# rensonnetg/microstructure_fingerprinting

Hardware: AMD Instinct MI355X
Metric: voxels/sec, 2-fascicle exhaustive NNLS, 782-atom x 200-measurement dictionary (higher is better)
Workload: dtype f64 (pairs ranked on split-f16 MFMA, short list re-evaluated in f64); 1 GPU; C2: 100000 voxels/GPU, 2 fascicles, 782 atoms x 200 measurements; voxels_per_gpu=100000, global_voxels=100000, atoms=782, measurements=200, ranks_in_group=1

## Files before the change

### microstructure_fingerprinting_amd/csrc/fit_k2.hip

```cpp
#pragma once
#include <type_traits>

#include "mfx_device.h"
#include "nnls_small.h"

typedef double d4 __attribute__((ext_vector_type(4)));

#define MFX_WG 512
#define MFX_MAXC 256
#define MFX_S_CAP 2048
#define MFX_DET_REL 1e-8
#define MFX_A12_REL 4e-14

struct FitK2Args {
  TablesDev T;
  PlanDev P;
  const double* Y;
  const double* peaks;
  int peaks_ld;
  const int* vox_list;
  const int* list_count;
  double* params;
  int num_params;
  int maxfasc;
  int csf_on, ear_on;
  unsigned long long* stamps;
  int* fb_count;
  int* fb_list;
  int maxc;
  int scap;
  const double* xc;
  struct Cand* xl_cand;
  int* xl_cnt;
  double* xl_mrg;
  int xl_cap;
  int vox_base;
  int* audit;
};

#ifdef MFX_STAMPS
#define MFX_STAMP(i) do { if (a.stamps && tid == 0) a.stamps[(size_t)blockIdx.x * 16 + (i)] = __builtin_amdgcn_s_memtime(); } while (0)
#else
#define MFX_STAMP(i) do { } while (0)
#endif

struct Cand {
  double score;
  int i, j;
};

__device__ __forceinline__ double wave_max(double v) {
#pragma unroll
  for (int o = 32; o > 0; o >>= 1) v = fmax(v, __shfl_xor(v, o));
  return v;
}
__device__ __forceinline__ double wave_sum(double v) {
#pragma unroll
  for (int o = 32; o > 0; o >>= 1) v += __shfl_xor(v, o);
  return v;
}

template <int I, int N, typename F>
__device__ __forceinline__ void mfx_static_for(F&& f) {
  if constexpr (I < N) {
    f(std::integral_constant<int, I>{});
    mfx_static_for<I + 1, N>(f);
  }
}

template <int KSTEPS, bool BRACKET, bool PIPE, int NW = 8, int TILES = 2, int NBUF = 2>
__global__ __launch_bounds__(NW * 64, NW == 8 ? 2 : 1) void mfx_fit_k2_kernel(FitK2Args a) {
  constexpr bool FAST = PIPE && !BRACKET;
  constexpr int WG = NW * 64;
  static_assert(!FAST || (NW == 8 && TILES == 2 && NBUF == 2), "the pipelined path is written for 8 waves, 2 tiles, 2 buffers");
  static_assert(TILES == 1 || TILES == 2, "TILES");
  static_assert(NBUF == 1 || NBUF == 2, "NBUF");
  constexpr int MP = KSTEPS * 4;
  constexpr int MPS = ((MP + 15) / 16) * 16;
  extern __shared__ double smem[];
  const int tid = threadIdx.x, lane = tid & 63, wave = tid >> 6;
  const int lg = lane >> 4, lc = lane & 15;
  const int M = a.P.M, N = a.T.N, ldn = a.T.ldn;
  const int NP = ldn;
  const int ntiles = NP >> 4;
  const double2* __restrict__ tab = a.T.tab;
  if (a.list_count && (int)blockIdx.x >= *a.list_count) return;
  const int vox = a.vox_list ? a.vox_list[blockIdx.x] : blockIdx.x;

  double* sB = smem;
  double* s_y = sB + NBUF * TILES * MPS * 16;
  double* s_t0 = s_y + MP;
  double* s_t1 = s_t0 + 2 * MP;
  double* s_tG = s_t1 + (BRACKET ? 2 * MP : 0);
  double* s_dG = s_tG + (BRACKET ? MP : 0);
  double* s_A11 = s_dG + (BRACKET ? MP : 0);
  double* s_Y1 = s_A11 + NP;
  double* s_A22 = s_Y1 + NP;
  double* s_Y2 = s_A22 + NP;
  double* s_S2 = s_Y2 + NP;
  double* s_S1 = s_S2 + NP;
  double* s_red = s_S1 + NP;
  Cand* s_cand = (Cand*)(s_red + 32);
  int* s_r0 = (int*)(s_cand + MFX_MAXC);
  int* s_r1 = s_r0 + 2 * MP;
  int* s_cnt = s_r1 + (BRACKET ? 2 * MP : 0);

  MFX_STAMP(0);
  const double* __restrict__ yv = a.Y + (size_t)vox * M;
  const double* __restrict__ pk = a.peaks + (size_t)vox * a.peaks_ld;
  for (int m = tid; m < MP; m += WG) s_y[m] = (m < M) ? yv[m] : 0.0;
  for (int idx = tid; idx < 2 * MP; idx += WG) {
    const int k = idx / MP, m = idx - k * MP;
    RowDesc rd;
    rd.r0 = a.T.P; rd.t0 = 0.0; rd.r1 = -1; rd.t1 = 0.0;
    if (m < M) rd = mfx_row_desc(a.T, a.P, m, pk[3 * k], pk[3 * k + 1], pk[3 * k + 2]);
    s_r0[idx] = rd.r0;
    s_t0[idx] = rd.t0;
    if (BRACKET) {
      s_r1[idx] = rd.r1;
      s_t1[idx] = rd.t1;
      if (k == 0) { s_tG[m] = (m < M) ? a.P.tG[m] : 0.0; s_dG[m] = (m < M) ? a.P.dG[m] : 1.0; }
    }
  }
  if (tid == 0) s_cnt[0] = 0;
  if (tid < 2) mfx_check_dir(a.P, pk + 3 * tid, vox);
  __syncthreads();

  auto elem = [&](int k, int m, int n) -> double {
    if (BRACKET) {
      RowDesc rd;
      rd.r0 = s_r0[k * MP + m]; rd.t0 = s_t0[k * MP + m];
      rd.r1 = s_r1[k * MP + m]; rd.t1 = s_t1[k * MP + m];
      return mfx_eval_br(tab, ldn, rd, s_tG[m], s_dG[m], n);
    } else {
      return mfx_eval(tab, ldn, s_r0[k * MP + m], s_t0[k * MP + m], n);
    }
  };

  MFX_STAMP(1);
  double y_sq = 0.0;
  for (int m = 0; m < M; ++m) y_sq += s_y[m] * s_y[m];
  double my_s[2] = {0.0, 0.0};
  int my_n[2] = {0, 0};
  for (int col = tid; col < 2 * NP; col += WG) {
    const int k = col >= NP, n = col - k * NP;
    double a2 = 0.0, ay = 0.0;
    if (n < N) {
#pragma unroll 8
      for (int m = 0; m < M; ++m) {
        if constexpr (FAST) {
          const double2 e = tab[(size_t)s_r0[k * MP + m] * ldn + n];
          const double d = fma(e.y, s_t0[k * MP + m], e.x);
          a2 = fma(d, d, a2);
          ay = fma(s_y[m], d, ay);
        } else {
          const double d = elem(k, m, n);
          a2 += d * d;
          ay += s_y[m] * d;
        }
      }
    }
    if constexpr (FAST) {
      const double inv = (n < N && a2 > 0.0) ? 1.0 / sqrt(a2) : 0.0;
      const double z = ay * inv;
      (k ? s_A22 : s_A11)[n] = inv;
      (k ? s_Y2 : s_Y1)[n] = z;
      const double s = z > 0.0 ? z * z : 0.0;
      if (s > my_s[k]) { my_s[k] = s; my_n[k] = n; }
    } else {
      (k ? s_A22 : s_A11)[n] = a2;
      (k ? s_Y2 : s_Y1)[n] = ay;
      const double s = (n < N && ay > 0.0) ? (ay * ay) / a2 : 0.0;
      (k ? s_S2 : s_S1)[n] = s;
      if (s > my_s[k]) { my_s[k] = s; my_n[k] = n; }
    }
  }
  const double eps_abs = 1e-9 * y_sq;
  double glb_run = 0.0;
  {
    double* s_bs = s_red;
    int* s_bn = (int*)(s_red + 16);
#pragma unroll
    for (int k = 0; k < 2; ++k) {
      double s = my_s[k];
      int n = my_n[k];
#pragma unroll
      for (int o = 32; o > 0; o >>= 1) {
        const double s2 = __shfl_xor(s, o);
        const int n2 = __shfl_xor(n, o);
        const bool take = (s2 > s) || (s2 == s && n2 < n);
// ... 422 lines not shown
```

### microstructure_fingerprinting_amd/csrc/fit_k2s.hip

```cpp
#pragma once
#include "fit_k2.hip"

typedef _Float16 h8 __attribute__((ext_vector_type(8)));
typedef _Float16 h4 __attribute__((ext_vector_type(4)));
typedef float f32x16 __attribute__((ext_vector_type(16)));
typedef float f32x2 __attribute__((ext_vector_type(2)));
typedef float f32x4 __attribute__((ext_vector_type(4)));
typedef int i32x4 __attribute__((ext_vector_type(4)));

#ifndef MFX_S_DC
#define MFX_S_DC 1.5e-5
#endif
template <int KS>
__host__ __device__ constexpr double mfx_s_dc() { return KS <= 13 ? (double)MFX_S_DC : 1.05 * (2.38e-6 + 3.0 * KS * 3.046e-7); }
#define MFX_S_DENMIN 1e-3
#define MFX_S_BOUND 0x40000000
#define MFX_S_GUARD 0.25

__device__ __forceinline__ unsigned long long mfx_nonneg_bits(double x) {
  return (unsigned long long)__double_as_longlong(x > 0.0 ? x : 0.0);
}

template <int CTRL>
__device__ __forceinline__ float mfx_dpp_max_f32(float v) {
  const int o = __builtin_amdgcn_update_dpp(0, __float_as_int(v), CTRL, 0xf, 0xf, false);
  return fmaxf(v, __int_as_float(o));
}
__device__ __forceinline__ double mfx_wave_max_down(double x) {
  float v = (float)x * (1.0f - 1.2e-7f);
  v = mfx_dpp_max_f32<0xb1>(v);
  v = mfx_dpp_max_f32<0x4e>(v);
  v = mfx_dpp_max_f32<0x141>(v);
  v = mfx_dpp_max_f32<0x140>(v);
  const int b = __float_as_int(v);
  const float r0 = __int_as_float(__builtin_amdgcn_readlane(b, 0)), r1 = __int_as_float(__builtin_amdgcn_readlane(b, 16)),
              r2 = __int_as_float(__builtin_amdgcn_readlane(b, 32)), r3 = __int_as_float(__builtin_amdgcn_readlane(b, 48));
  return (double)fmaxf(fmaxf(r0, r1), fmaxf(r2, r3));
}
__device__ __forceinline__ double mfx_rcp_nr(double x) {
  const double r0 = (double)__builtin_amdgcn_rcpf((float)x);
  return fma(r0, fma(-x, r0, 1.0), r0);
}

__device__ __forceinline__ double mfx_readlane_f64(double v, int l) {
  const long long b = __double_as_longlong(v);
  const unsigned lo = (unsigned)__builtin_amdgcn_readlane((int)(b & 0xffffffffll), l);
  const unsigned hi = (unsigned)__builtin_amdgcn_readlane((int)(b >> 32), l);
  return __longlong_as_double((long long)(((unsigned long long)hi << 32) | lo));
}

__device__ __forceinline__ void mfx_split16(float f, _Float16& hi, _Float16& lo) {
  asm("" : "+v"(f));
  const float h = __uint_as_float(__float_as_uint(f) & 0xffffe000u);
  hi = (_Float16)h;
  lo = (_Float16)(f - h);
}

#include "k2s_shared.h"

template <int KS, bool BR = false, int NB = 3, bool XC = false>
__global__ __launch_bounds__(512, 2) void mfx_fit_k2s_kernel(FitK2Args a) {
  constexpr int WG = 512, NW = 8;
  constexpr int MP = KS * 16;
  extern __shared__ double smem[];
  int tid = threadIdx.x;
  const int lane = tid & 63, wave = tid >> 6;
  const int lr = lane & 31, lh = lane >> 5;
  [[maybe_unused]] const int M = a.P.M;
  const int N = a.T.N, ldn = a.T.ldn;
  const int NP = (N + 31) & ~31;
  const int ntiles = NP >> 5;
  const int vox = a.vox_list ? a.vox_list[a.vox_base + blockIdx.x] : a.vox_base + (int)blockIdx.x;

  const K2sLds<KS, NB, BR, XC, NW * 64> L(smem, NP);
  K2S_UNPACK(L);
  const K2sVoxel VX = k2s_prologue<KS, NB, BR, XC, NW * 64, WG>(a, L, vox, tid);
  const double y_sq = VX.y_sq, yx = VX.yx, ramp = VX.ramp, dc_eff = VX.dc_eff, mrg = VX.mrg, etol = VX.etol;
  (void)y_sq; (void)yx;
  const float2* __restrict__ tab32 = a.P.tab32s;
  auto tab32_at = [&](int ro, int n) -> float2 { return *(const float2*)((const char*)tab32 + ((unsigned)(ro + n) << 3)); };
  auto tab32x2_at = [&](int ro, int n) -> f32x4 { return *(const f32x4*)((const char*)tab32 + ((unsigned)(ro + n) << 3)); };
  auto push = [&](double S, int i, int j) { k2s_push(L, a.scap, S, i, j); };

  MFX_STAMP(2);
#ifdef MFX_STAMPS_RND
  if (a.stamps && tid == 0) a.stamps[(size_t)blockIdx.x * 16] = __builtin_amdgcn_s_memtime();
#endif
  double bs1 = 0.0;
  int bn1 = 0;
  const int nrounds = (ntiles + NW - 1) / NW;
#ifdef MFX_EXP_NOAUDIT
  const int aud_key = -1;
#else
  const int aud_key = a.audit ? k2s_audit_key(k2s_audit_hash(vox), (ntiles % NW == 1 && ntiles > 1) ? ntiles - 1 : ntiles, ntiles) : -1;
#endif
  for (int round = 0; round < nrounds; ++round) {
    const bool tail = (ntiles - round * NW == 1) && (ntiles > 1);
    const int rt = tail ? round * NW : round * NW + wave;
    const bool rt_valid = rt < ntiles;
    const int rtc = rt_valid ? rt : 0;
    h8 afh[KS], afl[KS];
    {
      const int n = rtc * 32 + lr;
      const int nn = min(n, ldn - 1);
      double a2 = 0.0, ay = 0.0;
      float um1 = 0.0f;
      if constexpr (XC) um1 = (rt_valid && n < N) ? -s_uf[n] : 0.0f;
      mfx_static_for<0, KS>([&](auto kc) {
        constexpr int ks = decltype(kc)::value;
        float2 d[8];
#pragma unroll
        for (int j = 0; j < 8; ++j) d[j] = tab32_at(s_rs[16 * ks + 8 * lh + j], nn);
        h8 vh, vl;
#pragma unroll
        for (int j = 0; j < 8; ++j) {
          float fv = fmaf(d[j].y, s_t0f[16 * ks + 8 * lh + j], d[j].x);
          fv = rt_valid ? fv : 0.0f;
          if constexpr (XC) {
            if constexpr (ks == KS - 1) { if (j == 7) fv = lh ? um1 : fv; }
          } else {
            const double fd = (double)fv;
            a2 = fma(fd, fd, a2);
            ay = fma((double)s_yf[16 * ks + 8 * lh + j], fd, ay);
          }
          _Float16 x, y;
          mfx_split16(fv, x, y);
          vh[j] = x; vl[j] = y;
        }
        asm volatile("" : "+v"(vh), "+v"(vl));
        afh[ks] = vh; afl[ks] = vl;
        __builtin_amdgcn_sched_barrier(0);
      });
      if constexpr (!XC) {
      a2 += __shfl_xor(a2, 32);
      ay += __shfl_xor(ay, 32);
      const bool act = rt_valid && n < N;
      const double nrm = sqrt(a2);
      const double inv = (act && a2 > 0.0) ? 1.0 / nrm : 0.0;
      const double z = ay * inv;
      if (rt_valid && lh == 0) {
        s_Zf[n] = act ? (float)z : -1e30f;
        s_cs[n] = (act && a2 > 0.0) ? (float)nrm : 0.0f;
      }
      double sb = (act && z > 0.0) ? z * z : 0.0;
      int nb = n;
#pragma unroll
      for (int o = 16; o > 0; o >>= 1) {
        const double s2 = __shfl_xor(sb, o);
        const int n2 = __shfl_xor(nb, o);
        const bool take = (s2 > sb) || (s2 == sb && n2 < nb);
        sb = take ? s2 : sb;
        nb = take ? n2 : nb;
      }
      sb = mfx_readlane_f64(sb, 0);
      nb = __builtin_amdgcn_readfirstlane(nb);
      if (sb > bs1 || (sb == bs1 && sb > 0.0 && nb < bn1)) { bs1 = sb; bn1 = nb; }
      if (lane == 0 && sb - mrg > 0.0) atomicMax(&s_thr[0], mfx_nonneg_bits(sb - mrg));
      }
    }

    double thr = 0.0, thr_rows = -1.0;
#ifdef MFX_STAMPS_RND
    int dbg_flagged = 0, dbg_groups = 0;
#endif
    const float DCF = XC ? (float)((mfx_s_dc<KS>() + 2e-6) * ramp) * (1.0f + 2e-7f)
                         : (float)mfx_s_dc<KS>() + 2e-6f;
    auto pq_of = [&](float z, float rth, float& P, float& Q) {
      P = fminf(1.0f, fmaxf(z, 0.0f) * rth);
      Q = __builtin_amdgcn_sqrtf(fmaxf(0.0f, fmaf(-P, P, 1.0f) - 1.2e-7f)) * (1.0f - 3e-7f);
    };
    unsigned long long sc_thr = 0ull;
    float sc_z2 = 0.0f, sc_s = 0.0f;
    auto scan_pre = [&](int ct) {
      const int j = ct * 32 + lr;
      sc_thr = s_thr[0];
      sc_z2 = s_Zf[NP + j];
      sc_s = s_cs[NP + j];
    };
#ifdef MFX_STAMPS_SCAN
    int dbg_calls = 0;
#define MFX_SCAN_T(k) do { if (a.stamps && round == 0 && dbg_calls == 1 && wave == 0 && lane == 0) a.stamps[(size_t)blockIdx.x * 16 + (k)] = __builtin_amdgcn_s_memtime(); } while (0)
#else
#define MFX_SCAN_T(k) do { } while (0)
#endif
    auto scan_main = [&](const f32x16& acc, int ct) {
#ifdef MFX_STAMPS_SCAN
      ++dbg_calls;
#endif
      MFX_SCAN_T(0);
      {
        if (((rt << 8) | ct) == aud_key) {
          const unsigned h = k2s_audit_hash(vox);
          const int ga = (h >> 16) & 15;
          float v = acc[0];
#pragma unroll
          for (int g = 1; g < 16; ++g) v = (ga == g) ? acc[g] : v;
          if (lane == (int)((h >> 20) & 63)) ((float*)(s_red + 30))[0] = v;
        }
      }
      const int j = ct * 32 + lr;
      thr = fmax(thr, __longlong_as_double((long long)sc_thr));
      const float rth = __builtin_amdgcn_rsqf(fmaxf((float)thr * (1.0f - 2e-7f), 1e-30f)) * (1.0f + 4e-7f);
      float* pqw = s_pq + wave * 64;
      if (thr > thr_rows) {
        thr_rows = thr;
        if (lane < 32) {
          const float z1 = s_Zf[rtc * 32 + lane], n1 = s_cs[rtc * 32 + lane];
          float P, Q;
          pq_of(z1, rth, P, Q);
          const bool ok = n1 > 0.0f;
          pqw[lane] = ok ? (P + DCF) * n1 : 0.0f;
          pqw[32 + lane] = ok ? Q * ((1.0f - DCF) * n1) : 1e18f;
        }
      }
      const float z2f = sc_z2, n2 = sc_s;
      float P2, Q2;
      pq_of(z2f, rth, P2, Q2);
      const bool colok = n2 > 0.0f;
      const float p2 = colok ? (P2 + DCF) * n2 : -1e18f, q2 = colok ? Q2 * ((1.0f - DCF) * n2) : 1e18f;
      float mm[4];
#pragma unroll
      for (int q = 0; q < 4; ++q) {
        const f32x4 p1q = *(const f32x4*)(pqw + 8 * q + 4 * lh);
        const f32x4 q1q = *(const f32x4*)(pqw + 32 + 8 * q + 4 * lh);
        float t[4];
#pragma unroll
        for (int u = 0; u < 4; ++u) t[u] = fmaf(-q1q[u], q2, fmaf(p1q[u], p2, -acc[4 * q + u]));
        mm[q] = fmaxf(fmaxf(t[0], t[1]), fmaxf(t[2], t[3]));
      }
      MFX_SCAN_T(1);
      if (__any(fmaxf(fmaxf(mm[0], mm[1]), fmaxf(mm[2], mm[3])) >= 0.0f)) {
        MFX_SCAN_T(2);
#ifdef MFX_STAMPS_RND
        ++dbg_flagged;
#endif
        const double z2 = (double)s_Zf[NP + j], n2d = (double)s_cs[NP + j];
#pragma unroll 1
        for (int q = 0; q < 4; ++q) {
          if (!__any(mm[q] >= 0.0f)) continue;
          const f32x4 p1q = *(const f32x4*)(pqw + 8 * q + 4 * lh);
          const f32x4 q1q = *(const f32x4*)(pqw + 32 + 8 * q + 4 * lh);
#pragma unroll 1
          for (int gg = 0; gg < 4; ++gg) {
            const int g = 4 * q + gg;
            if (!__any(fmaf(-q1q[gg], q2, fmaf(p1q[gg], p2, -acc[g])) >= 0.0f)) continue;
#ifdef MFX_STAMPS_RND
            ++dbg_groups;
#endif
            const int i = rt * 32 + (g & 3) + 8 * (g >> 2) + 4 * lh;
            const double n12 = (double)s_cs[i] * n2d;
            const double c = n12 > 0.0 ? (double)acc[g] * mfx_rcp_nr(n12) : 0.0;
            const double z1 = (double)s_Zf[i];
            const double e1 = fma(-c, z2, z1);
            const double e2 = fma(-c, z1, z2);
            const double den = fma(-c, c, 1.0);
            const double num = fma(z2, e2, z1 * e1);
            const bool pos = (e1 > -etol) & (e2 > -etol);
            const bool wellc = (den >= MFX_S_DENMIN) & (c >= 0.0);
            const bool hit = pos & wellc & (fma(-thr, den, num) >= 0.0);
            const bool near = pos & !wellc;
            if (!__any(hit | near)) continue;
            double S = -1.0;
            if (hit) {
              S = num * mfx_rcp_nr(den);
            } else if (near) {
              const double dlo = den - 2.0 * dc_eff - dc_eff * dc_eff;
              const double u1 = fabs(e1) + etol, u2 = fabs(e2) + etol;
              S = (dlo > 0.0 && c > -0.5) ? fmin(fma(z2, z2, u1 * u1 / dlo), fma(z1, z1, u2 * u2 / dlo)) + mrg : 1e300;
            }
            bool feas = hit;
            double q1x = 0.0, q2x = 0.0;
            if constexpr (XC) {
              q1x = (double)s_uf[i] * mfx_rcp_nr(fmax((double)s_cs[i], 1e-300));
              q2x = (double)s_uf[NP + j] * mfx_rcp_nr(fmax(n2d, 1e-300));
              feas = hit && (fma(-e2, q2x, fma(-e1, q1x, yx * den)) >= 8.0 * etol);
            }
            double sraise = feas ? S : 0.0;
            double slist = S;
            if constexpr (XC) {
              if (__any(hit && !feas)) {
                const double n1p = (double)s_cs[i], u1 = (double)s_uf[i], u2 = (double)s_uf[NP + j];
                const double m1 = fma(u1, u1, n1p * n1p), m2 = fma(u2, u2, n2d * n2d);
                const double i1 = mfx_rcp_nr(fmax(sqrt(m1), 1e-300)), i2 = mfx_rcp_nr(fmax(sqrt(m2), 1e-300));
                const double w1 = fma(u1, yx, z1 * n1p) * i1, w2 = fma(u2, yx, z2 * n2d) * i2;
                const double c0 = fma(u1, u2, (double)acc[g]) * i1 * i2;
                const double f1 = fma(-c0, w2, w1), f2 = fma(-c0, w1, w2), den0 = fma(-c0, c0, 1.0);
                const bool ok0 = hit && !feas && (f1 > etol) && (f2 > etol) && (den0 >= MFX_S_DENMIN) && (c0 >= 0.0) && (m1 > 0.0) && (m2 > 0.0);
                if (ok0) sraise = fma(w2, f2, w1 * f1) * mfx_rcp_nr(den0) - yx * yx;
                const bool xneg = hit && (e1 > etol) && (e2 > etol) && (fma(-e2, q2x, fma(-e1, q1x, yx * den)) <= -8.0 * etol) &&
                                  (den0 >= MFX_S_DENMIN) && (c0 >= 0.0) && (m1 > 0.0) && (m2 > 0.0);
                if (xneg) {
                  if (ok0) slist = sraise + mrg;
                  else if (f1 < -etol || f2 < -etol) slist = -1.0;
                }
              }
            }
            const double smax = mfx_wave_max_down(fmax(sraise, 0.0));
            if (smax - 2.0 * mrg > thr) {
              thr = smax - 2.0 * mrg;
              if (lane == 0) atomicMax(&s_thr[0], mfx_nonneg_bits(thr));
            }
            if ((hit | near) && slist >= thr) push(slist, i, hit ? j : (j | MFX_S_BOUND));
#ifdef MFX_STAMPS_SCAN
            if (a.stamps && round == 0 && dbg_calls == 1 && wave == 0 && lane == 0) {
              unsigned long long* st = a.stamps + (size_t)blockIdx.x * 16;
              if (st[15] < 8) st[4 + st[15]] = __builtin_amdgcn_s_memtime();
              ++st[15];
            }
#endif
          }
        }
        MFX_SCAN_T(3);
      }
    };
    auto scan_tile = [&](const f32x16& acc, int ct) { scan_pre(ct); scan_main(acc, ct); };

#ifdef MFX_EXP_NOTAIL
    if (tail) continue;
#endif
    if (tail) {
#ifdef MFX_STAMPS_RND
      if (a.stamps && tid == 0 && round < 4) a.stamps[(size_t)blockIdx.x * 16 + 2 * round + 1] = __builtin_amdgcn_s_memtime();
#endif
      thr = __longlong_as_double((long long)s_thr[0]);
      for (int ct = wave; ct < ntiles; ct += NW) {
        const int n = ct * 32 + lr;
        const int nn = min(n, ldn - 1);
        float tail_u2 = 0.0f;
        if constexpr (XC) tail_u2 = s_uf[NP + n];
        f32x16 acc;
#pragma unroll
        for (int g = 0; g < 16; ++g) acc[g] = 0.0f;
        float2 d[2][8];
#pragma unroll
        for (int j = 0; j < 8; ++j) d[0][j] = tab32_at(s_rs[MP + 8 * lh + j], nn);
        mfx_static_for<0, KS>([&](auto kc) {
          constexpr int ks = decltype(kc)::value;
          if constexpr (ks + 1 < KS) {
#pragma unroll
            for (int j = 0; j < 8; ++j) d[(ks + 1) & 1][j] = tab32_at(s_rs[MP + 16 * (ks + 1) + 8 * lh + j], nn);
          }
          h8 bh, bl;
#pragma unroll
          for (int j = 0; j < 8; ++j) {
            _Float16 x, y;
            float fv = fmaf(d[ks & 1][j].y, s_t0f[MP + 16 * ks + 8 * lh + j], d[ks & 1][j].x);
            if constexpr (XC && ks == KS - 1) { if (j == 7) fv = lh ? tail_u2 : fv; }
            mfx_split16(fv, x, y);
            bh[j] = x; bl[j] = y;
          }
          acc = __builtin_amdgcn_mfma_f32_32x32x16_f16(afh[ks], bh, acc, 0, 0, 0);
          acc = __builtin_amdgcn_mfma_f32_32x32x16_f16(afh[ks], bl, acc, 0, 0, 0);
          acc = __builtin_amdgcn_mfma_f32_32x32x16_f16(afl[ks], bh, acc, 0, 0, 0);
          __builtin_amdgcn_sched_barrier(0);
        });
        scan_tile(acc, ct);
      }
      __syncthreads();
#ifdef MFX_STAMPS_RND
      if (a.stamps && tid == 0 && round < 4) a.stamps[(size_t)blockIdx.x * 16 + 2 * round + 2] = __builtin_amdgcn_s_memtime();
#endif
      continue;
    }

    const int grp = wave >> 2, tg = tid & 255;
    static_assert(KS <= 16, "one generation item per thread");
    f32x4 gd[8];
    const int gq = KS * grp + (tg >> 4);
    const bool gact = (tg >> 4) < KS;
    auto gen_load = [&](int ch) {
      const int nn = min(ch * 32 + 2 * (tg & 15), ldn - 2);
      const int q = gact ? gq : KS * grp;
#pragma unroll
      for (int e = 0; e < 8; ++e) gd[e] = tab32x2_at(s_rs[MP + 8 * q + e], nn);
    };
#ifndef MFX_XC_GT
#define MFX_XC_GT 0
#endif
    constexpr bool GT = KS <= 13 && (!XC || MFX_XC_GT);
    float g_t[GT ? 8 : 1];
    if constexpr (GT) {
#pragma unroll
      for (int e = 0; e < 8; ++e) g_t[e] = s_t0f[MP + 8 * (gact ? gq : KS * grp) + e];
    }
    auto gen_store = [&](int ch, int buf) {
      if (gact) {
        const int c0 = 2 * (tg & 15);
        h8 hi0, lo0, hi1, lo1;
        float gu0 = 0.0f, gu1 = 0.0f;
        if constexpr (XC) { gu0 = s_uf[NP + ch * 32 + c0]; gu1 = s_uf[NP + ch * 32 + c0 + 1]; }
#pragma unroll
        for (int e = 0; e < 8; ++e) {
          const float t = GT ? g_t[GT ? e : 0] : s_t0f[MP + 8 * gq + e];
          _Float16 x, y;
          float v0 = fmaf(gd[e][1], t, gd[e][0]), v1 = fmaf(gd[e][3], t, gd[e][2]);
          if constexpr (XC) { if (e == 7) { const bool spare = (gq == 2 * KS - 1); v0 = spare ? gu0 : v0; v1 = spare ? gu1 : v1; } }
          mfx_split16(v0, x, y);
          hi0[e] = x; lo0[e] = y;
          mfx_split16(v1, x, y);
          hi1[e] = x; lo1[e] = y;
        }
        const int off = (gq * 32 + c0) << 3;
        _Float16* dh = sBh + buf * KS * 512 + off;
        _Float16* dl = sBl + buf * KS * 512 + off;
        *(h8*)dh = hi0; *(h8*)(dh + 8) = hi1;
        *(h8*)dl = lo0; *(h8*)(dl + 8) = lo1;
      }
    };
    f32x16 acc;
#pragma unroll
    for (int g = 0; g < 16; ++g) acc[g] = 0.0f;
    auto mfma_chunk = [&](int buf) {
#pragma unroll
      for (int g = 0; g < 16; ++g) acc[g] = 0.0f;
      const _Float16* bhp = sBh + buf * KS * 512 + lane * 8;
      const _Float16* blp = sBl + buf * KS * 512 + lane * 8;
      h8 bh = *(const h8*)bhp, bl = *(const h8*)blp;
      mfx_static_for<0, KS>([&](auto kc) {
        constexpr int ks = decltype(kc)::value;
        h8 bhn = bh, bln = bl;
        if constexpr (ks + 1 < KS) {
          bhn = *(const h8*)(bhp + (ks + 1) * 512);
          bln = *(const h8*)(blp + (ks + 1) * 512);
        }
        acc = __builtin_amdgcn_mfma_f32_32x32x16_f16(afh[ks], bh, acc, 0, 0, 0);
        acc = __builtin_amdgcn_mfma_f32_32x32x16_f16(afh[ks], bl, acc, 0, 0, 0);
        acc = __builtin_amdgcn_mfma_f32_32x32x16_f16(afl[ks], bh, acc, 0, 0, 0);
        bh = bhn; bl = bln;
        __builtin_amdgcn_sched_barrier(0);
      });
    };

    if (round == 0) MFX_STAMP(3);
#ifdef MFX_STAMPS_RND
    if (a.stamps && tid == 0 && round < 4) a.stamps[(size_t)blockIdx.x * 16 + 2 * round + 1] = __builtin_amdgcn_s_memtime();
#endif
    if constexpr (NB == 3) {
      gen_load(0);
      gen_store(0, 0);
      if (grp == 0) {
        if (ntiles > 1) { gen_load(1); gen_store(1, 1); }
        if (ntiles > 2) gen_load(2);
      } else if (ntiles > 1) {
        gen_load(1);
      }
      __syncthreads();
      if (round == 0) MFX_STAMP(4);
      thr = __longlong_as_double((long long)s_thr[0]);
      int b0 = 0;
#ifdef MFX_EXP_NOGEN
      const bool exp_gen = round == 0;
#else
      constexpr bool exp_gen = true;
#endif
      for (int c = 0; c <= ntiles; ++c) {
#ifdef MFX_STAMPS_HS
#ifndef MFX_HS_ROUND
#define MFX_HS_ROUND 1
#define MFX_HS_C0 10
#endif
        if (a.stamps && round == MFX_HS_ROUND && c >= MFX_HS_C0 && c < MFX_HS_C0 + 16 && tid == 0) a.stamps[(size_t)blockIdx.x * 16 + c - MFX_HS_C0] = __builtin_amdgcn_s_memtime();
#endif
        const int b1 = b0 == 2 ? 0 : b0 + 1, b2 = b1 == 2 ? 0 : b1 + 1;
        if (grp == 0) {
          if (c < ntiles) {
            if (rt_valid) { mfma_chunk(b0); scan_pre(c); }
            if (exp_gen && c + 2 < ntiles) gen_store(c + 2, b2);
            if (rt_valid) scan_main(acc, c);
            if (exp_gen && c + 3 < ntiles) gen_load(c + 3);
          }
        } else {
          if (c >= 1 && rt_valid) scan_pre(c - 1);
          if (exp_gen && c + 1 < ntiles) gen_store(c + 1, b1);
          if (c >= 1 && rt_valid) scan_main(acc, c - 1);
          if (exp_gen && c + 2 < ntiles) gen_load(c + 2);
          if (c < ntiles && rt_valid) mfma_chunk(b0);
        }
// ... 36 lines not shown
```

### microstructure_fingerprinting_amd/csrc/k2s_launch.h

```cpp
#pragma once
#include "mfx_host.h"
#include "fit_k2s.hip"

template <int KS, bool BR, int NB>
static int launch_k2s_t(const FitK2Args& a, int nvox, hipStream_t st) {
  MfxThread& T = mfx_thread();
  const size_t lds = mfx_k2s_lds_bytes(KS, a.T.N, BR, NB);
  auto kern = mfx_fit_k2s_kernel<KS, BR, NB>;
  HIPCHK(hipFuncSetAttribute((const void*)kern, hipFuncAttributeMaxDynamicSharedMemorySize, (int)lds));
  StreamMem fbm(st);
  HIPCHK(fbm.alloc(sizeof(int) * ((size_t)nvox + 8)));
  int* fb = fbm.as<int>();
  HIPCHK(hipMemsetAsync(fb, 0, 8 * sizeof(int), st));
  if (int rc = mfx_prof_begin(st)) return rc;
  FitK2Args aa = a;
  aa.stamps = T.stamps;
  aa.fb_count = fb;
  aa.fb_list = fb + 8;
  aa.audit = fb + 2;
  aa.scap = T.k2s_cap ? T.k2s_cap : MFX_S_CAP;
  hipLaunchKernelGGL(kern, dim3(nvox), dim3(512), lds, st, aa);
  HIPCHK(hipGetLastError());
  if (int rc = mfx_prof_end(st)) return rc;
  FitK2Args ab = a;
  ab.vox_list = fb + 8;
  ab.list_count = fb;
  if (int rc = mfx_launch_k2_f64(ab, nvox, st, false)) return rc;
  if (int rc = mfx_fb_accumulate(fb, 2, st)) return rc;
  return mfx_fb_accumulate_audit(fb + 2, st);
}

#define MFX_K2S_TU(KS_, NAME_)                                                            \
  int NAME_(const FitK2Args& a, int nvox, hipStream_t st, bool br, int NB) {              \
    if (NB == 3) return br ? launch_k2s_t<KS_, true, 3>(a, nvox, st) : launch_k2s_t<KS_, false, 3>(a, nvox, st); \
    return br ? launch_k2s_t<KS_, true, 2>(a, nvox, st) : launch_k2s_t<KS_, false, 2>(a, nvox, st);              \
  }
```

### microstructure_fingerprinting_amd/csrc/k2s_shared.h

```cpp
#pragma once

template <int KS, int NB, bool BR, bool XC, int PQF>
struct K2sLds {
  static constexpr int MP = KS * 16;
  double* smem;
  _Float16* sBh;
  _Float16* sBl;
  double* s_y;
  double* s_t0;
  double* s_red;
  Cand* s_cand;
  unsigned long long* s_thr;
  int* s_r0;
  int* s_cnt;
  float* s_t0f;
  float* s_Zf;
  float* s_cs;
  float* s_yf;
  float* s_pq;
  double* s_t1;
  double* s_tG;
  double* s_dG;
  int* s_r1;
  int* s_rs;
  int* s_evl4;
  float* s_xf;
  float* s_uf;
  __device__ __forceinline__ K2sLds(double* smem_, int NP) : smem(smem_) {
    sBh = (_Float16*)smem;
    sBl = sBh + NB * KS * 512;
    s_y = (double*)(sBl + NB * KS * 512);
    s_t0 = s_y + MP;
    s_red = s_t0 + 2 * MP;
    s_cand = (Cand*)(s_red + 32);
    s_thr = (unsigned long long*)(s_cand + MFX_S_CAP);
    s_r0 = (int*)(s_thr + 2);
    s_cnt = s_r0 + 2 * MP;
    s_t0f = (float*)(s_cnt + 4);
    s_Zf = s_t0f + 2 * MP;
    s_cs = s_Zf + 2 * NP;
    s_yf = s_cs + 2 * NP;
    s_pq = s_yf + MP;
    s_t1 = (double*)(s_pq + PQF);
    s_tG = s_t1 + (BR ? 2 * MP : 0);
    s_dG = s_tG + (BR ? MP : 0);
    s_r1 = (int*)(s_dG + (BR ? MP : 0));
    s_rs = BR ? s_r1 + 2 * MP : s_r0;
    s_evl4 = s_r1 + (BR ? 4 * MP : 0);
    s_xf = (float*)(s_evl4 + (KS < 8 ? MFX_S_CAP : 0));
    s_uf = s_xf + (XC ? MP : 0);
  }
};
#define K2S_UNPACK(L) \
  [[maybe_unused]] _Float16* const sBh = (L).sBh; \
  [[maybe_unused]] _Float16* const sBl = (L).sBl; \
  [[maybe_unused]] double* const s_y = (L).s_y; \
  [[maybe_unused]] double* const s_t0 = (L).s_t0; \
  [[maybe_unused]] double* const s_red = (L).s_red; \
  [[maybe_unused]] Cand* const s_cand = (L).s_cand; \
  [[maybe_unused]] unsigned long long* const s_thr = (L).s_thr; \
  [[maybe_unused]] int* const s_r0 = (L).s_r0; \
  [[maybe_unused]] int* const s_cnt = (L).s_cnt; \
  [[maybe_unused]] float* const s_t0f = (L).s_t0f; \
  [[maybe_unused]] float* const s_Zf = (L).s_Zf; \
  [[maybe_unused]] float* const s_cs = (L).s_cs; \
  [[maybe_unused]] float* const s_yf = (L).s_yf; \
  [[maybe_unused]] float* const s_pq = (L).s_pq; \
  [[maybe_unused]] double* const s_t1 = (L).s_t1; \
  [[maybe_unused]] double* const s_tG = (L).s_tG; \
  [[maybe_unused]] double* const s_dG = (L).s_dG; \
  [[maybe_unused]] int* const s_r1 = (L).s_r1; \
  [[maybe_unused]] int* const s_rs = (L).s_rs; \
  [[maybe_unused]] int* const s_evl4 = (L).s_evl4; \
  [[maybe_unused]] float* const s_xf = (L).s_xf; \
  [[maybe_unused]] float* const s_uf = (L).s_uf;

struct K2sVoxel {
  double y_sq;
  double yx;
  double ramp;
  double dc_eff;
  double mrg;
  double etol;
};

__device__ __forceinline__ unsigned k2s_audit_hash(int vox) {
  unsigned h = (unsigned)vox * 2654435761u;
  h ^= h >> 15; h *= 2246822519u; h ^= h >> 13; h *= 3266489917u; h ^= h >> 16;
  return h;
}
__device__ __forceinline__ int k2s_audit_key(unsigned h, int ntiles_reg, int ntiles) {
  return ntiles_reg > 0 ? (int)(((h & 0xffu) % (unsigned)ntiles_reg) << 8) | (int)(((h >> 8) & 0xffu) % (unsigned)ntiles) : -1;
}

template <class LDS>
__device__ __forceinline__ void k2s_push(const LDS& L, int scap, double S, int i, int j) {
  const int slot = atomicAdd(&L.s_cnt[0], 1);
  const int idx = slot & (scap - 1);
  if (slot >= scap) {
    const double old = L.s_cand[idx].score;
    atomicMax(&L.s_thr[1], mfx_nonneg_bits(fmin(old, 1e300)));
  }
  L.s_cand[idx].score = S;
  L.s_cand[idx].i = i;
  L.s_cand[idx].j = j;
}

template <int KS, int NB, bool BR, bool XC, int PQF, int WG>
__device__ __forceinline__ K2sVoxel k2s_prologue(const FitK2Args& a, const K2sLds<KS, NB, BR, XC, PQF>& L, const int vox, const int tid) {
  constexpr int MP = KS * 16, NW = WG / 64;
  const int lane = tid & 63, wave = tid >> 6;
  const int M = a.P.M, N = a.T.N, ldn = a.T.ldn;
  const int NP = (N + 31) & ~31;
  [[maybe_unused]] double* const smem = L.smem;
  K2S_UNPACK(L);

  MFX_STAMP(0);
  const double* __restrict__ yv = a.Y + (size_t)vox * M;
  const double* __restrict__ pk = a.peaks + (size_t)vox * a.peaks_ld;
  for (int m = tid; m < MP; m += WG) { const double v = (m < M) ? yv[m] : 0.0; s_y[m] = v; s_yf[m] = (float)v; }
  for (int idx = tid; idx < 2 * MP; idx += WG) {
    const int k = idx / MP, m = idx - k * MP;
    RowDesc rd;
    rd.r0 = a.T.P; rd.t0 = 0.0; rd.r1 = -1; rd.t1 = 0.0;
    if (m < M) rd = mfx_row_desc(a.T, a.P, m, pk[3 * k], pk[3 * k + 1], pk[3 * k + 2]);
    s_r0[idx] = rd.r0 * ldn;
    s_t0[idx] = rd.t0;
    if constexpr (!BR) {
      s_t0f[idx] = (float)rd.t0;
    } else {
      s_r1[idx] = rd.r1 < 0 ? -1 : rd.r1 * ldn;
      s_t1[idx] = rd.t1;
      if (k == 0) { s_tG[m] = (m < M) ? a.P.tG[m] : 0.0; s_dG[m] = (m < M) ? a.P.dG[m] : 1.0; }
      int rs = a.T.P;
      double ts = 0.0;
      if (m < M) {
        const int sg = a.P.s_scr[m], st = a.P.offs[2 * sg], cn = a.P.offs[2 * sg + 1];
        const double u = mfx_absdot(a.P.g + 3 * m, pk[3 * k], pk[3 * k + 1], pk[3 * k + 2]);
        int j = mfx_searchsorted_left(a.P.xs + st, cn, u);
        j = j < 1 ? 1 : (j > cn - 1 ? cn - 1 : j);
        rs = st + j - 1;
        ts = u - a.P.xs[rs];
      }
      s_rs[idx] = rs * ldn;
      s_t0f[idx] = (float)ts;
    }
  }
  if (tid == 0) { s_cnt[0] = 0; s_cnt[1] = 0; s_thr[0] = 0ull; s_thr[1] = 0ull; ((float*)(s_red + 30))[0] = __int_as_float(0x7fc00000); }
  if constexpr (XC) {
    for (int m = tid; m < MP; m += WG) s_xf[m] = (m < M) ? (float)a.xc[m] : 0.0f;
    if (tid < 2) ((unsigned long long*)s_red)[24 + tid] = 0ull;
  }
  if (tid < 2) mfx_check_dir(a.P, pk + 3 * tid, vox);
  __syncthreads();

  const float2* __restrict__ tab32 = a.P.tab32s;
  auto tab32x2_at = [&](int ro, int n) -> f32x4 { return *(const f32x4*)((const char*)tab32 + ((unsigned)(ro + n) << 3)); };

  MFX_STAMP(1);
  double y_sq_v = 0.0;
  for (int m = 0; m < M; ++m) y_sq_v += s_y[m] * s_y[m];
  const double y_sq = mfx_readlane_f64(y_sq_v, 0);
  double rsh_v = 1.0, yx_v = 0.0;
  if constexpr (XC) {
    double h = 0.0, xy = 0.0;
    for (int m = 0; m < M; ++m) { const double xv = (double)s_xf[m]; h = fma(xv, xv, h); xy = fma(xv, (double)s_yf[m], xy); }
    rsh_v = h > 0.0 ? 1.0 / sqrt(h) : 0.0;
    yx_v = xy * rsh_v;
  }
  const double rsh = mfx_readlane_f64(rsh_v, 0), yx = mfx_readlane_f64(yx_v, 0);
  const double y_sq_p = XC ? fmax(y_sq - yx * yx, 0.0) : y_sq;
  double my_s[2] = {0.0, 0.0};
  int my_n[2] = {0, 0};
  {
    const int VH = ((N + 1) / 2 + 63) & ~63;
    const int npass = (VH + WG - 1) / WG;
#pragma unroll 1
    for (int kd = XC ? 0 : 1; kd < 2; ++kd) {
    double ms_cur = 0.0, rm2_cur = 1.0;
    int mn_cur = 0;
    for (int p0 = 0; p0 < npass; p0 += 2) {
      int kq[2], nq[2];
      bool wact[2];
      double a2[2][2], ay[2][2], au[2][2];
#pragma unroll
      for (int q = 0; q < 2; ++q) {
        const int v = tid + WG * (p0 + q);
        kq[q] = kd;
        nq[q] = 2 * v;
        wact[q] = __any((p0 + q < npass) && (nq[q] < N));
        a2[q][0] = a2[q][1] = ay[q][0] = ay[q][1] = 0.0;
        au[q][0] = au[q][1] = 0.0;
      }
      int ncl[2];
#pragma unroll
      for (int q = 0; q < 2; ++q) ncl[q] = min(nq[q], ldn - 2);
      f32x4 dbuf[2][2][4];
      auto issue = [&](int m4, auto stc) {
        constexpr int st = decltype(stc)::value;
#pragma unroll
        for (int q = 0; q < 2; ++q) {
          if (wact[q]) {
            const i32x4 r = *(const i32x4*)(s_rs + kq[q] * MP + m4);
#pragma unroll
            for (int e = 0; e < 4; ++e) dbuf[st][q][e] = tab32x2_at(r[e], ncl[q]);
          }
        }
      };
      auto accumulate = [&](int m4, auto stc) {
        constexpr int st = decltype(stc)::value;
        const f32x4 yv = *(const f32x4*)(s_yf + m4);
        f32x4 xv = {0.0f, 0.0f, 0.0f, 0.0f};
        if constexpr (XC) xv = *(const f32x4*)(s_xf + m4);
#pragma unroll
        for (int q = 0; q < 2; ++q) {
          if (wact[q]) {
            const f32x4 t = *(const f32x4*)(s_t0f + kq[q] * MP + m4);
#pragma unroll
            for (int e = 0; e < 4; ++e) {
              const f32x4 d = dbuf[st][q][e];
              const double d0 = (double)fmaf(d[1], t[e], d[0]), d1 = (double)fmaf(d[3], t[e], d[2]);
              const double ye = (double)yv[e];
              a2[q][0] = fma(d0, d0, a2[q][0]);
              ay[q][0] = fma(ye, d0, ay[q][0]);
              a2[q][1] = fma(d1, d1, a2[q][1]);
              ay[q][1] = fma(ye, d1, ay[q][1]);
              if constexpr (XC) {
                const double xe = (double)xv[e];
                au[q][0] = fma(xe, d0, au[q][0]);
                au[q][1] = fma(xe, d1, au[q][1]);
              }
            }
          }
        }
      };
      issue(0, std::integral_constant<int, 0>{});
      for (int m4 = 0; m4 < MP; m4 += 8) {
        issue(m4 + 4, std::integral_constant<int, 1>{});
        accumulate(m4, std::integral_constant<int, 0>{});
        if (m4 + 8 < MP) issue(m4 + 8, std::integral_constant<int, 0>{});
        accumulate(m4 + 4, std::integral_constant<int, 1>{});
      }
#pragma unroll
      for (int q = 0; q < 2; ++q) {
#pragma unroll
        for (int u = 0; u < 2; ++u) {
          const int k = kq[q], n = nq[q] + u;
          if (p0 + q < npass && n < NP) {
            const bool act = n < N;
            if constexpr (!XC) {
              const double inv = (act && a2[q][u] > 0.0) ? 1.0 / sqrt(a2[q][u]) : 0.0;
              const double z = ay[q][u] * inv;
              s_Zf[k * NP + n] = act ? (float)z : -1e30f;
              s_cs[NP + n] = (act && inv > 0.0) ? (float)sqrt(a2[q][u]) : 0.0f;
              const double s = z > 0.0 ? z * z : 0.0;
              if (act && s > ms_cur) { ms_cur = s; mn_cur = n; }
            } else {
              const double uu = au[q][u] * rsh;
              const double n2p = a2[q][u] - uu * uu;
              const bool ok = act && a2[q][u] > 0.0;
              if (ok && !(n2p > a2[q][u] * (1.0 / 16.0))) s_cnt[1] = 1;
              const bool okp = ok && n2p > 0.0;
              const double np = okp ? sqrt(n2p) : 0.0;
              const double inv = okp ? 1.0 / np : 0.0;
              const double z = (ay[q][u] - uu * yx) * inv;
              s_Zf[k * NP + n] = act ? (float)z : -1e30f;
              s_cs[k * NP + n] = okp ? (float)np : 0.0f;
              s_uf[k * NP + n] = okp ? (float)uu : 0.0f;
              if (okp) rm2_cur = fmax(rm2_cur, a2[q][u] * inv * inv);
              const bool feas = okp && z > 0.0 && (yx - z * inv * uu) >= 0.0;
              const double s = feas ? z * z : 0.0;
              if (s > ms_cur) { ms_cur = s; mn_cur = n; }
            }
          }
        }
      }
    }
    if (kd == 0) { my_s[0] = ms_cur; my_n[0] = mn_cur; } else { my_s[1] = ms_cur; my_n[1] = mn_cur; }
    if constexpr (XC) {
      if (rm2_cur > 1.0) atomicMax((unsigned long long*)s_red + 24 + kd, mfx_nonneg_bits(rm2_cur));
    }
    }
  }
  {
    double* s_bs = s_red;
    int* s_bn = (int*)(s_red + 16);
#pragma unroll
    for (int k = XC ? 0 : 1; k < 2; ++k) {
      double s = my_s[k];
      int n = my_n[k];
#pragma unroll
      for (int o = 32; o > 0; o >>= 1) {
        const double s2 = __shfl_xor(s, o);
        const int n2 = __shfl_xor(n, o);
        const bool take = (s2 > s) || (s2 == s && n2 < n);
        s = take ? s2 : s;
        n = take ? n2 : n;
      }
      if (lane == 0) { s_bs[k * 8 + wave] = s; s_bn[k * 8 + wave] = n; }
    }
    __syncthreads();
  }
  double ramp_v = 1.0;
  if constexpr (XC) {
    const unsigned long long* rw = (const unsigned long long*)s_red + 24;
    ramp_v = sqrt(fmax(1.0, __longlong_as_double((long long)rw[0]))) * sqrt(fmax(1.0, __longlong_as_double((long long)rw[1])));
  }
  const double ramp = mfx_readlane_f64(ramp_v, 0);
  const double dc_eff = XC ? mfx_s_dc<KS>() * ramp : mfx_s_dc<KS>();
  const double mrg = mfx_readlane_f64(XC ? fmax(dc_eff * y_sq_p + 2e-6 * ramp * sqrt(y_sq * y_sq_p), 1e-9 * y_sq) : dc_eff * y_sq_p, 0);
  const double etol = mfx_readlane_f64(XC ? dc_eff * sqrt(y_sq_p) + 2e-6 * ramp * sqrt(y_sq) : dc_eff * sqrt(y_sq_p), 0);
  {
    double* s_bs = s_red;
    int* s_bn = (int*)(s_red + 16);
    if (tid == 0) {
      double best1 = 0.0;
      for (int k = XC ? 0 : 1; k < 2; ++k) {
        double s = s_bs[k * 8];
        int n = s_bn[k * 8];
        for (int w = 1; w < NW; ++w) {
          const double s2 = s_bs[k * 8 + w];
          const int n2 = s_bn[k * 8 + w];
          if (s2 > s || (s2 == s && n2 < n)) { s = s2; n = n2; }
        }
        best1 = fmax(best1, s);
        if (!XC && s > 0.0) {
          const int slot = s_cnt[0]++;
          s_cand[slot].score = s + mrg;
          s_cand[slot].i = k ? 0 : n;
          s_cand[slot].j = (k ? n : 0) | MFX_S_BOUND;
        }
// ... 394 lines not shown
```

Measured before the change: 1.093 million voxels/s.

## Fuse tail-tile MFMA with second-fascicle stats and park accumulators in slab

With 782 atoms there are 25 tiles of 32, and 25 % 8 == 1, so the last round is a single-row tail. For that case the kernel now computes the tail row's A fragments first and runs the tail MFMAs across all waves. That pass is merged with the second-fascicle column statistics (norms, correlations, best single atom) that the prologue used to compute separately. The resulting accumulators are parked in a global scratch slab, claimed per block with a CAS on a flag array, and read back in the tail round for scanning. This removes a redundant pass over the dictionary and the serial tail generation. In exchange it adds global-memory round trips, slot contention, and a fallback path that sends the voxel to the fallback list when no slot is free.

After: 1.104 million voxels/s (median of 6 runs). Within noise of the previous version (+1.0%).

```diff
diff --git a/microstructure_fingerprinting_amd/csrc/fit_k2.hip b/microstructure_fingerprinting_amd/csrc/fit_k2.hip
--- a/microstructure_fingerprinting_amd/csrc/fit_k2.hip
+++ b/microstructure_fingerprinting_amd/csrc/fit_k2.hip
@@ -36,6 +36,9 @@
   int xl_cap;
   int vox_base;
   int* audit;
+  float* slab;
+  int* slab_flags;
+  int slab_slots;
 };
 
 #ifdef MFX_STAMPS
diff --git a/microstructure_fingerprinting_amd/csrc/fit_k2s.hip b/microstructure_fingerprinting_amd/csrc/fit_k2s.hip
--- a/microstructure_fingerprinting_amd/csrc/fit_k2s.hip
+++ b/microstructure_fingerprinting_amd/csrc/fit_k2s.hip
@@ -57,6 +57,22 @@
 }
 
 #include "k2s_shared.h"
+
+__device__ __forceinline__ int mfx_xor_i32(int v, int ln, int o) { return __builtin_amdgcn_ds_bpermute((ln ^ o) << 2, v); }
+__device__ __forceinline__ double mfx_xor_f64(double v, int ln, int o) {
+  const long long b = __double_as_longlong(v);
+  const unsigned lo = (unsigned)mfx_xor_i32((int)(b & 0xffffffffll), ln, o), hi = (unsigned)mfx_xor_i32((int)(b >> 32), ln, o);
+  return __longlong_as_double((long long)(((unsigned long long)hi << 32) | lo));
+}
+
+__device__ __forceinline__ int k2s_slab_claim(int* flags, int S, unsigned b) {
+  int s = (int)(b % (unsigned)S);
+  for (int k = 0; k < 64 * S; ++k) {
+    if (atomicCAS(&flags[s], 0, 1) == 0) return s;
+    s = (s + 1 == S) ? 0 : s + 1;
+  }
+  return -1;
+}
 
 template <int KS, bool BR = false, int NB = 3, bool XC = false>
 __global__ __launch_bounds__(512, 2) void mfx_fit_k2s_kernel(FitK2Args a) {
@@ -74,18 +90,25 @@
 
   const K2sLds<KS, NB, BR, XC, NW * 64> L(smem, NP);
   K2S_UNPACK(L);
-  const K2sVoxel VX = k2s_prologue<KS, NB, BR, XC, NW * 64, WG>(a, L, vox, tid);
+#ifdef MFX_STAMPS_RND
+  if (a.stamps && tid == 0) a.stamps[(size_t)blockIdx.x * 16 + 12] = __builtin_amdgcn_s_memtime();
+#endif
+  const bool fused = !XC && (ntiles % NW == 1) && ntiles > 1;
+  if (fused && tid == WG - 64) ((int*)(s_red + 28))[0] = k2s_slab_claim(a.slab_flags, a.slab_slots, blockIdx.x);
+  const K2sVoxel VX = k2s_prologue<KS, NB, BR, XC, NW * 64, WG>(a, L, vox, tid, !fused);
   const double y_sq = VX.y_sq, yx = VX.yx, ramp = VX.ramp, dc_eff = VX.dc_eff, mrg = VX.mrg, etol = VX.etol;
   (void)y_sq; (void)yx;
   const float2* __restrict__ tab32 = a.P.tab32s;
   auto tab32_at = [&](int ro, int n) -> float2 { return *(const float2*)((const char*)tab32 + ((unsigned)(ro + n) << 3)); };
   auto tab32x2_at = [&](int ro, int n) -> f32x4 { return *(const f32x4*)((const char*)tab32 + ((unsigned)(ro + n) << 3)); };
   auto push = [&](double S, int i, int j) { k2s_push(L, a.scap, S, i, j); };
+  const int slot = fused ? __builtin_amdgcn_readfirstlane(((const int*)(s_red + 28))[0]) : -1;
+  if (fused && slot < 0) {
+    if (tid == 0) a.fb_list[atomicAdd(a.fb_count, 1)] = vox;
+    return;
+  }
 
   MFX_STAMP(2);
-#ifdef MFX_STAMPS_RND
-  if (a.stamps && tid == 0) a.stamps[(size_t)blockIdx.x * 16] = __builtin_amdgcn_s_memtime();
-#endif
   double bs1 = 0.0;
   int bn1 = 0;
   const int nrounds = (ntiles + NW - 1) / NW;
@@ -94,70 +117,169 @@
 #else
   const int aud_key = a.audit ? k2s_audit_key(k2s_audit_hash(vox), (ntiles % NW == 1 && ntiles > 1) ? ntiles - 1 : ntiles, ntiles) : -1;
 #endif
+  auto gen_a = [&](const int rtc, const bool rt_valid, h8 (&afh)[KS], h8 (&afl)[KS]) {
+    int ln = lane;
+    asm volatile("" : "+v"(ln));
+    const int n = rtc * 32 + lr;
+    const int nn = min(n, ldn - 1);
+    double a2 = 0.0, ay = 0.0;
+    float um1 = 0.0f;
+    if constexpr (XC) um1 = (rt_valid && n < N) ? -s_uf[n] : 0.0f;
+    mfx_static_for<0, KS>([&](auto kc) {
+      constexpr int ks = decltype(kc)::value;
+      float2 d[8];
+#pragma unroll
+      for (int j = 0; j < 8; ++j) d[j] = tab32_at(s_rs[16 * ks + 8 * lh + j], nn);
+      h8 vh, vl;
+#pragma unroll
+      for (int j = 0; j < 8; ++j) {
+        float fv = fmaf(d[j].y, s_t0f[16 * ks + 8 * lh + j], d[j].x);
+        fv = rt_valid ? fv : 0.0f;
+        if constexpr (XC) {
+          if constexpr (ks == KS - 1) { if (j == 7) fv = lh ? um1 : fv; }
+        } else {
+          const double fd = (double)fv;
+          a2 = fma(fd, fd, a2);
+          ay = fma((double)s_yf[16 * ks + 8 * lh + j], fd, ay);
+        }
+        _Float16 x, y;
+        mfx_split16(fv, x, y);
+        vh[j] = x; vl[j] = y;
+      }
+      asm volatile("" : "+v"(vh), "+v"(vl));
+      afh[ks] = vh; afl[ks] = vl;
+      __builtin_amdgcn_sched_barrier(0);
+    });
+    if constexpr (!XC) {
+    a2 += mfx_xor_f64(a2, ln, 32);
+    ay += mfx_xor_f64(ay, ln, 32);
+    const bool act = rt_valid && n < N;
+    const double nrm = sqrt(a2);
+    const double inv = (act && a2 > 0.0) ? 1.0 / nrm : 0.0;
+    const double z = ay * inv;
+    if (rt_valid && lh == 0) {
+      s_Zf[n] = act ? (float)z : -1e30f;
+      s_cs[n] = (act && a2 > 0.0) ? (float)nrm : 0.0f;
+    }
+    double sb = (act && z > 0.0) ? z * z : 0.0;
+    int nb = n;
+#pragma unroll
+    for (int o = 16; o > 0; o >>= 1) {
+      const double s2 = mfx_xor_f64(sb, ln, o);
+      const int n2 = mfx_xor_i32(nb, ln, o);
+      const bool take = (s2 > sb) || (s2 == sb && n2 < nb);
+      sb = take ? s2 : sb;
+      nb = take ? n2 : nb;
+    }
+    sb = mfx_readlane_f64(sb, 0);
+    nb = __builtin_amdgcn_readfirstlane(nb);
+    if (sb > bs1 || (sb == bs1 && sb > 0.0 && nb < bn1)) { bs1 = sb; bn1 = nb; }
+    if (lane == 0 && sb - mrg > 0.0) atomicMax(&s_thr[0], mfx_nonneg_bits(sb - mrg));
+    }
+  };
+  if (fused) {
+    h8 afh[KS], afl[KS];
+    gen_a(ntiles - 1, true, afh, afl);
+#ifdef MFX_STAMPS_RND
+    if (a.stamps && tid == 0) a.stamps[(size_t)blockIdx.x * 16 + 13] = __builtin_amdgcn_s_memtime();
+#endif
+    const int npark = (N - 32 * (ntiles - 1)) <= 16 ? 2 : 4;
+    f32x4* __restrict__ park = (f32x4*)(a.slab + (size_t)slot * (size_t)ntiles * 1024) + lane;
+    double ms = 0.0;
+    int mn = 0;
+    int ln = lane;
+    asm volatile("" : "+v"(ln));
+    for (int ct = wave; ct < ntiles; ct += NW) {
+      const int n = ct * 32 + lr;
+      const int nn = min(n, ldn - 1);
+      f32x16 acc;
+#pragma unroll
+      for (int g = 0; g < 16; ++g) acc[g] = 0.0f;
+      double a2 = 0.0, ay = 0.0;
+      float2 d[2][8];
+#pragma unroll
+      for (int j = 0; j < 8; ++j) d[0][j] = tab32_at(s_rs[MP + 8 * lh + j], nn);
+      mfx_static_for<0, KS>([&](auto kc) {
+        constexpr int ks = decltype(kc)::value;
+        if constexpr (ks + 1 < KS) {
+#pragma unroll
+          for (int j = 0; j < 8; ++j) d[(ks + 1) & 1][j] = tab32_at(s_rs[MP + 16 * (ks + 1) + 8 * lh + j], nn);
+        }
+        h8 bh, bl;
+#pragma unroll
+        for (int j = 0; j < 8; ++j) {
+          const float fv = fmaf(d[ks & 1][j].y, s_t0f[MP + 16 * ks + 8 * lh + j], d[ks & 1][j].x);
+          const double fd = (double)fv;
+          a2 = fma(fd, fd, a2);
+          ay = fma((double)s_yf[16 * ks + 8 * lh + j], fd, ay);
+          _Float16 x, y;
+          mfx_split16(fv, x, y);
+          bh[j] = x; bl[j] = y;
+        }
+#ifndef MFX_EXP_NOTAIL
+        acc = __builtin_amdgcn_mfma_f32_32x32x16_f16(afh[ks], bh, acc, 0, 0, 0);
+        acc = __builtin_amdgcn_mfma_f32_32x32x16_f16(afh[ks], bl, acc, 0, 0, 0);
+        acc = __builtin_amdgcn_mfma_f32_32x32x16_f16(afl[ks], bh, acc, 0, 0, 0);
+#else
+        (void)bh; (void)bl;
+#endif
+        __builtin_amdgcn_sched_barrier(0);
+      });
+      a2 += mfx_xor_f64(a2, ln, 32);
+      ay += mfx_xor_f64(ay, ln, 32);
+      const bool act = n < N;
+      const double inv = (act && a2 > 0.0) ? 1.0 / sqrt(a2) : 0.0;
+      const double z = ay * inv;
+      if (lh == 0) {
+        s_Zf[NP + n] = act ? (float)z : -1e30f;
+        s_cs[NP + n] = (act && inv > 0.0) ? (float)sqrt(a2) : 0.0f;
+      }
+      const double sz = z > 0.0 ? z * z : 0.0;
+      if (act && sz > ms) { ms = sz; mn = n; }
+#ifndef MFX_EXP_NOTAIL
+#pragma unroll
+      for (int q = 0; q < 4; ++q)
+        if (q < npark) park[(ct * 4 + q) * 64] = f32x4{acc[4 * q], acc[4 * q + 1], acc[4 * q + 2], acc[4 * q + 3]};
+#endif
+    }
+    double* s_bs = s_red;
+    int* s_bn = (int*)(s_red + 16);
+#pragma unroll
+    for (int o = 32; o > 0; o >>= 1) {
+      const double s2 = mfx_xor_f64(ms, ln, o);
+      const int n2 = mfx_xor_i32(mn, ln, o);
+      const bool take = (s2 > ms) || (s2 == ms && n2 < mn);
+      ms = take ? s2 : ms;
+      mn = take ? n2 : mn;
+    }
+    if (lane == 0) { s_bs[wave] = ms; s_bn[wave] = mn; }
+    __syncthreads();
+    if (tid == 0) {
+      double sb = s_bs[0];
+      int nb = s_bn[0];
+      for (int w = 1; w < NW; ++w) {
+        const double s2 = s_bs[w];
+        const int n2 = s_bn[w];
+        if (s2 > sb || (s2 == sb && n2 < nb)) { sb = s2; nb = n2; }
+      }
+      if (sb > 0.0) {
+        push(sb + mrg, 0, nb | MFX_S_BOUND);
+        atomicMax(&s_thr[0], mfx_nonneg_bits(sb - mrg));
+      }
+    }
+    bs1 = mfx_readlane_f64(bs1, 0);
+    bn1 = __builtin_amdgcn_readfirstlane(bn1);
+  }
+#ifdef MFX_STAMPS_RND
+  if (a.stamps && tid == 0) a.stamps[(size_t)blockIdx.x * 16] = __builtin_amdgcn_s_memtime();
+#endif
   for (int round = 0; round < nrounds; ++round) {
     const bool tail = (ntiles - round * NW == 1) && (ntiles > 1);
     const int rt = tail ? round * NW : round * NW + wave;
     const bool rt_valid = rt < ntiles;
     const int rtc = rt_valid ? rt : 0;
     h8 afh[KS], afl[KS];
-    {
-      const int n = rtc * 32 + lr;
-      const int nn = min(n, ldn - 1);
-      double a2 = 0.0, ay = 0.0;
-      float um1 = 0.0f;
-      if constexpr (XC) um1 = (rt_valid && n < N) ? -s_uf[n] : 0.0f;
-      mfx_static_for<0, KS>([&](auto kc) {
-        constexpr int ks = decltype(kc)::value;
-        float2 d[8];
-#pragma unroll
-        for (int j = 0; j < 8; ++j) d[j] = tab32_at(s_rs[16 * ks + 8 * lh + j], nn);
-        h8 vh, vl;
-#pragma unroll
-        for (int j = 0; j < 8; ++j) {
-          float fv = fmaf(d[j].y, s_t0f[16 * ks + 8 * lh + j], d[j].x);
-          fv = rt_valid ? fv : 0.0f;
-          if constexpr (XC) {
-            if constexpr (ks == KS - 1) { if (j == 7) fv = lh ? um1 : fv; }
-          } else {
-            const double fd = (double)fv;
-            a2 = fma(fd, fd, a2);
-            ay = fma((double)s_yf[16 * ks + 8 * lh + j], fd, ay);
-          }
-          _Float16 x, y;
-          mfx_split16(fv, x, y);
-          vh[j] = x; vl[j] = y;
-        }
-        asm volatile("" : "+v"(vh), "+v"(vl));
-        afh[ks] = vh; afl[ks] = vl;
-        __builtin_amdgcn_sched_barrier(0);
-      });
-      if constexpr (!XC) {
-      a2 += __shfl_xor(a2, 32);
-      ay += __shfl_xor(ay, 32);
-      const bool act = rt_valid && n < N;
-      const double nrm = sqrt(a2);
-      const double inv = (act && a2 > 0.0) ? 1.0 / nrm : 0.0;
-      const double z = ay * inv;
-      if (rt_valid && lh == 0) {
-        s_Zf[n] = act ? (float)z : -1e30f;
-        s_cs[n] = (act && a2 > 0.0) ? (float)nrm : 0.0f;
-      }
-      double sb = (act && z > 0.0) ? z * z : 0.0;
-      int nb = n;
-#pragma unroll
-      for (int o = 16; o > 0; o >>= 1) {
-        const double s2 = __shfl_xor(sb, o);
-        const int n2 = __shfl_xor(nb, o);
-        const bool take = (s2 > sb) || (s2 == sb && n2 < nb);
-        sb = take ? s2 : sb;
-        nb = take ? n2 : nb;
-      }
-      sb = mfx_readlane_f64(sb, 0);
-      nb = __builtin_amdgcn_readfirstlane(nb);
-      if (sb > bs1 || (sb == bs1 && sb > 0.0 && nb < bn1)) { bs1 = sb; bn1 = nb; }
-      if (lane == 0 && sb - mrg > 0.0) atomicMax(&s_thr[0], mfx_nonneg_bits(sb - mrg));
-      }
-    }
+    if (XC || !tail) gen_a(rtc, rt_valid, afh, afl);
 
     double thr = 0.0, thr_rows = -1.0;
 #ifdef MFX_STAMPS_RND
@@ -316,13 +438,36 @@
     auto scan_tile = [&](const f32x16& acc, int ct) { scan_pre(ct); scan_main(acc, ct); };
 
 #ifdef MFX_EXP_NOTAIL
-    if (tail) continue;
+    if (XC && tail) continue;
 #endif
     if (tail) {
 #ifdef MFX_STAMPS_RND
       if (a.stamps && tid == 0 && round < 4) a.stamps[(size_t)blockIdx.x * 16 + 2 * round + 1] = __builtin_amdgcn_s_memtime();
 #endif
       thr = __longlong_as_double((long long)s_thr[0]);
+      if constexpr (!XC) {
+#ifndef MFX_EXP_NOTAIL
+        const int npark = (N - 32 * (ntiles - 1)) <= 16 ? 2 : 4;
+        int pl = lane;
+        asm volatile("" : "+v"(pl));
+        const f32x4* __restrict__ park = (const f32x4*)(a.slab + (size_t)slot * (size_t)ntiles * 1024) + pl;
+        for (int ct = wave; ct < ntiles; ct += NW) {
+          f32x4 v[4];
+#pragma unroll
+          for (int q = 0; q < 4; ++q) v[q] = q < npark ? park[(ct * 4 + q) * 64] : f32x4{1e30f, 1e30f, 1e30f, 1e30f};
+          f32x16 acc;
+#pragma unroll
+          for (int g = 0; g < 16; ++g) acc[g] = v[g >> 2][g & 3];
+          scan_tile(acc, ct);
+        }
+#endif
+        __syncthreads();
+        if (tid == 0) atomicExch(&a.slab_flags[slot], 0);
+#ifdef MFX_STAMPS_RND
+        if (a.stamps && tid == 0 && round < 4) a.stamps[(size_t)blockIdx.x * 16 + 2 * round + 2] = __builtin_amdgcn_s_memtime();
+#endif
+        continue;
+      }
       for (int ct = wave; ct < ntiles; ct += NW) {
         const int n = ct * 32 + lr;
         const int nn = min(n, ldn - 1);
diff --git a/microstructure_fingerprinting_amd/csrc/k2s_launch.h b/microstructure_fingerprinting_amd/csrc/k2s_launch.h
--- a/microstructure_fingerprinting_amd/csrc/k2s_launch.h
+++ b/microstructure_fingerprinting_amd/csrc/k2s_launch.h
@@ -19,6 +19,22 @@
   aa.fb_list = fb + 8;
   aa.audit = fb + 2;
   aa.scap = T.k2s_cap ? T.k2s_cap : MFX_S_CAP;
+  StreamMem slab(st);
+  const int ntiles = (a.T.N + 31) / 32;
+  aa.slab = nullptr; aa.slab_flags = nullptr; aa.slab_slots = 0;
+  if (ntiles % 8 == 1 && ntiles > 1) {
+    int dev = 0, cus = 0, occ = 0;
+    HIPCHK(hipGetDevice(&dev));
+    HIPCHK(hipDeviceGetAttribute(&cus, hipDeviceAttributeMultiprocessorCount, dev));
+    HIPCHK(hipOccupancyMaxActiveBlocksPerMultiprocessor(&occ, (const void*)kern, 512, lds));
+    const int S = std::max(1, std::min(std::max(2, occ) * std::max(cus, 1), nvox));
+    const size_t slab_bytes = (size_t)S * (size_t)ntiles * 4096;
+    HIPCHK(slab.alloc(slab_bytes + sizeof(int) * (size_t)S));
+    aa.slab = slab.as<float>();
+    aa.slab_flags = (int*)((char*)slab.p + slab_bytes);
+    aa.slab_slots = S;
+    HIPCHK(hipMemsetAsync(aa.slab_flags, 0, sizeof(int) * (size_t)S, st));
+  }
   hipLaunchKernelGGL(kern, dim3(nvox), dim3(512), lds, st, aa);
   HIPCHK(hipGetLastError());
   if (int rc = mfx_prof_end(st)) return rc;
diff --git a/microstructure_fingerprinting_amd/csrc/k2s_shared.h b/microstructure_fingerprinting_amd/csrc/k2s_shared.h
--- a/microstructure_fingerprinting_amd/csrc/k2s_shared.h
+++ b/microstructure_fingerprinting_amd/csrc/k2s_shared.h
@@ -107,7 +107,8 @@
 }
 
 template <int KS, int NB, bool BR, bool XC, int PQF, int WG>
-__device__ __forceinline__ K2sVoxel k2s_prologue(const FitK2Args& a, const K2sLds<KS, NB, BR, XC, PQF>& L, const int vox, const int tid) {
+__device__ __forceinline__ K2sVoxel k2s_prologue(const FitK2Args& a, const K2sLds<KS, NB, BR, XC, PQF>& L, const int vox, const int tid,
+                                                 const bool stats_d2 = true) {
   constexpr int MP = KS * 16, NW = WG / 64;
   const int lane = tid & 63, wave = tid >> 6;
   const int M = a.P.M, N = a.T.N, ldn = a.T.ldn;
@@ -175,8 +176,9 @@
   {
     const int VH = ((N + 1) / 2 + 63) & ~63;
     const int npass = (VH + WG - 1) / WG;
+    const int kd_end = (XC || stats_d2) ? 2 : 1;
 #pragma unroll 1
-    for (int kd = XC ? 0 : 1; kd < 2; ++kd) {
+    for (int kd = XC ? 0 : 1; kd < kd_end; ++kd) {
     double ms_cur = 0.0, rm2_cur = 1.0;
     int mn_cur = 0;
     for (int p0 = 0; p0 < npass; p0 += 2) {
```
